# LeoQLi/DeepSIR

Hardware: AMD Instinct MI355X
Metric: registered pairs/sec (5k-pt 3DMatch-shaped synthetic pairs, 5 registration iterations, KNN pyramid included) (higher is better)
Workload: dtype f32 (GEMMs as fp16-pair MFMA, fp32 accumulate; index decisions exact fp32)

## Files before the change

### deepsir_amd/_lib.py

```python
from __future__ import annotations

import ctypes as C
import os

_HERE = os.path.dirname(os.path.abspath(__file__))
LIB_PATH = os.environ.get("DSIR_LIB", os.path.join(_HERE, "libdsir.so"))

c_float_p = C.POINTER(C.c_float)
c_i32_p = C.POINTER(C.c_int32)
c_i64_p = C.POINTER(C.c_int64)


class dsir_cfg(C.Structure):
    _fields_ = [
        ("feat_len", C.c_int32),
        ("num_knn", C.c_int32),
        ("num_layers", C.c_int32),
        ("sub_sampling_ratio", C.c_int32 * 4),
        ("d_out", C.c_int32 * 4),
        ("out_feat_dim", C.c_int32),
        ("num_classes", C.c_int32),
        ("max_points", C.c_int32),
        ("max_pairs", C.c_int32),
        ("pipeline", C.c_int32),
# ... 39 lines not shown
        ("xyz", C.c_void_p), ("feat", C.c_void_p), ("logits", C.c_void_p), ("score", C.c_void_p), ("label", C.c_void_p),
        ("index", C.c_void_p),
    ]


SYMBOLS = {
    "dsir_create": (C.c_int, [C.c_int, C.POINTER(dsir_cfg), C.POINTER(C.c_void_p)]),
    "dsir_create_ex": (C.c_int, [C.c_int, C.POINTER(dsir_cfg), C.c_int, C.POINTER(C.c_void_p)]),
    "dsir_destroy": (None, [C.c_void_p]),
    "dsir_last_error": (C.c_char_p, [C.c_void_p]),
    "dsir_stream": (C.c_void_p, [C.c_void_p]),
    "dsir_sync": (C.c_int, [C.c_void_p]),
    "dsir_set_stream": (C.c_int, [C.c_void_p, C.c_void_p, C.c_int]),
    "dsir_num_weights": (C.c_int, [C.c_void_p]),
    "dsir_weight_name": (C.c_char_p, [C.c_void_p, C.c_int, c_i64_p]),
    "dsir_load_weight": (C.c_int, [C.c_void_p, C.c_char_p, C.c_void_p, c_i64_p, C.c_int]),
    "dsir_finalize_weights": (C.c_int, [C.c_void_p]),
    "dsir_narrow_i64": (C.c_int, [C.c_void_p, C.c_void_p, C.c_void_p, C.c_int64]),
    "dsir_knn_pyramid": (C.c_int, [C.c_void_p, C.c_void_p, C.c_int, C.c_int, C.c_int, C.c_void_p, C.c_void_p,
                                   C.c_void_p, C.c_void_p]),
    "dsir_randla_forward": (C.c_int, [C.c_void_p, C.c_int, C.c_void_p, C.c_int, C.c_int, C.c_int, C.c_void_p,
                                      C.c_void_p, C.c_void_p, C.c_void_p, C.c_void_p, C.c_void_p]),
    "dsir_lfa_enc2_probe": (C.c_int, [C.c_void_p, C.c_int, C.c_int, C.c_int, C.c_int, C.c_int, C.c_void_p, C.c_void_p, C.c_void_p, C.c_void_p]),
    "dsir_ppf_pre": (C.c_int, [C.c_void_p, C.c_int, C.c_void_p, C.c_int, C.c_void_p, C.c_int64, C.c_int, C.c_int, C.c_void_p]),
    "dsir_estimate_normals": (C.c_int, [C.c_void_p, C.c_void_p, C.c_int, C.c_void_p, C.c_int64, C.c_int, C.c_int, c_float_p, C.c_void_p,
                                        C.c_void_p]),
    "dsir_estimate_normals_csr": (C.c_int, [C.c_void_p, C.c_void_p, C.c_int, C.c_void_p, C.c_void_p, C.c_int, C.c_int, c_float_p, C.c_void_p,
                                            C.c_void_p]),
    "dsir_fpfh": (C.c_int, [C.c_void_p, C.c_void_p, C.c_int, C.c_void_p, C.c_void_p, C.c_int64, C.c_void_p, C.c_void_p, C.c_int, C.c_int,
                            C.c_void_p, C.c_int, C.c_void_p]),
    "dsir_iss_keypoints": (C.c_int, [C.c_void_p, C.c_void_p, C.c_int, C.c_void_p, C.c_void_p, C.c_void_p, C.c_void_p, C.c_int, C.c_int,
                                     C.c_double, C.c_double, C.c_int, C.c_void_p, C.c_void_p, C.c_void_p, C.c_void_p]),
    "dsir_score": (C.c_int, [C.c_void_p, C.c_void_p, C.c_void_p, C.c_void_p, C.c_int64, C.c_void_p, C.c_int64,
                             C.c_int, C.c_int, C.c_void_p, C.c_void_p]),
    "dsir_aggregate": (C.c_int, [C.c_void_p, C.c_void_p, C.c_int64, C.c_void_p, C.c_void_p, C.c_int, C.c_int,
                                 C.c_void_p]),
    "dsir_nn_match": (C.c_int, [C.c_void_p, C.c_void_p, C.c_void_p, C.c_int, C.c_int, C.c_int, C.c_void_p]),
    "dsir_nn_match_screened": (C.c_int, [C.c_void_p, C.c_void_p, C.c_void_p, C.c_int, C.c_int, C.c_int, C.c_void_p, c_i64_p]),
    "dsir_kabsch": (C.c_int, [C.c_void_p, C.c_void_p, C.c_void_p, C.c_void_p, C.c_int, C.c_int, C.c_void_p,
                              C.c_void_p]),
    "dsir_register": (C.c_int, [C.c_void_p, C.POINTER(dsir_pair_batch), C.c_int, C.POINTER(dsir_pair_result)]),
    "dsir_forward_pair": (C.c_int, [C.c_void_p, C.POINTER(dsir_pair_batch), C.c_int, C.POINTER(dsir_cloud_out),
                                    C.POINTER(dsir_cloud_out)]),
    "dsir_icp_refine": (C.c_int, [C.c_void_p, C.c_void_p, C.c_void_p, C.c_int, C.c_int, C.c_int, C.c_int, C.c_float, C.c_int,
                                  C.c_float, C.c_float, C.c_void_p, C.c_void_p, C.c_void_p]),
    "dsir_icp_refine_ex": (C.c_int, [C.c_void_p, C.c_void_p, C.c_void_p, C.c_int, C.c_int, C.c_int, C.c_int, C.c_float, C.c_int,
# ... 181 lines not shown
```

### deepsir_amd/csrc/build.py

```python
from __future__ import annotations

import os
import subprocess
import sys
from concurrent.futures import ThreadPoolExecutor

HERE = os.path.dirname(os.path.abspath(__file__))
PKG = os.path.dirname(HERE)
ROOT = os.path.dirname(PKG)
SOURCES = ["engine.hip", "register.hip", "entries_stage.hip", "entries_pose.hip", "weights.hip", "schedule.hip", "search.hip", "pw_gemm.hip", "pw_stream.hip", "pw_tile.hip", "walk.hip", "att_pool.hip", "lse_uv.hip", "head_mlp.hip", "agg_chain.hip", "select.hip", "misc.hip", "knn.hip", "knn_grid.hip", "score.hip", "nn_match.hip", "nn_screen.hip", "nn_prune.hip", "kabsch.hip", "icp.hip", "icp_grid.hip", "finetune.hip", "pose_corr.hip", "ransac.hip", "consensus.hip", "fgr.hip", "align_loss.hip", "train_gemm.hip", "train_norm.hip", "train_gather.hip", "train_loss.hip", "train_elem.hip", "match_targets.hip", "metrics.hip", "preprocess.hip", "augment.hip", "crop.hip", "ppf.hip", "fpfh.hip", "iss.hip", "overlap.hip", "radius_nn.hip", "nn_topk.hip", "resample.hip", "seg_sort.hip", "info_matrix.hip", "pose_graph.hip"]
HEADERS = ["kernels.h", "device_utils.h", "svd3.h", "split_f16.h", "agg_chain_body.h", "head_mlp_body.h", "pw_tile_body.h", "att_pool_body.h", "misc_body.h", "ppf_plan.h", "search_plan.h", "screen_bound.h", "exact_search_body.h", "icp_plane.h", "icp_robust.h", "icp_grid.h", "icp_layout.h", "cell_index.h", "radius_nn.h", "scratch.h", "op_layouts.h", "train_ops.h", "train_layouts.h", "seg_sort.h", "augment_params.h", "pose_corr.h", "fgr.h", "engine_ctx.h", "pose_graph.h", os.path.join(ROOT, "include", "dsir.h"), os.path.join(ROOT, "include", "dsir_train.h")]
OUT = os.path.join(PKG, "libdsir.so")
FLAGS = ["--offload-arch=gfx950", "-O3", "-std=c++17", "-fPIC", "-ffp-contract=off", "-I" + os.path.join(ROOT, "include"),
         "-I" + HERE, "-Wall", "-Wno-unused-function", "-Wno-unused-value"]


def _newer(target, deps):
    if not os.path.exists(target):
        return False
    t = os.path.getmtime(target)
    return all(os.path.getmtime(d) <= t for d in deps)


def build(force: bool = False, verbose: bool = False) -> str:
    hipcc = os.environ.get("HIPCC", "/opt/rocm/bin/hipcc")
    objdir = os.path.join(HERE, "build")
    os.makedirs(objdir, exist_ok=True)
    hdrs = [h if os.path.isabs(h) else os.path.join(HERE, h) for h in HEADERS]
    jobs = []
    for s in SOURCES:
        src = os.path.join(HERE, s)
        obj = os.path.join(objdir, s.replace(".hip", ".o"))
        if force or not _newer(obj, [src] + hdrs):
# ... 28 lines not shown
```

### deepsir_amd/csrc/engine_ctx.h

```cpp
#pragma once
#include <hip/hip_runtime.h>

#include <string>
#include <unordered_map>
#include <vector>

#include "dsir.h"
#include "kernels.h"
#include "search_plan.h"

namespace dsir {

struct HostParam {
  std::string name;
  std::vector<int64_t> shape;
  std::vector<float> data;
  bool loaded = false;
  bool ignored = false;
  int64_t numel() const { int64_t n = 1; for (auto s : shape) n *= s; return n; }
};

struct Mlp2dW { const float *W = nullptr, *b = nullptr, *gamma = nullptr, *beta = nullptr; int cin = 0, cout = 0, groups = 0; };
struct AttW { const float* fc = nullptr; const float* fc_g = nullptr; int d = 0; Mlp2dW mlp; };
struct BlockW { Mlp2dW mlp1, lfa1, lfa2, mlp2, skip; AttW att1, att2; int d_in = 0, d = 0; const float* lse_w8 = nullptr;
// ... 178 lines not shown
struct EncCache {
  bool valid = false;
  float* s2_buf[DSIR_MAX_LEVELS][2] = {};
  float* enc_buf[DSIR_MAX_LEVELS] = {};
  float* uv_buf[DSIR_MAX_LEVELS] = {};
  float* dist_buf[DSIR_MAX_LEVELS] = {};
  float* enc2_buf[DSIR_MAX_LEVELS] = {};
  double* enc_stats[DSIR_MAX_LEVELS] = {};
  double* enc2_stats[DSIR_MAX_LEVELS] = {};
  Act enc[DSIR_MAX_LEVELS], enc2[DSIR_MAX_LEVELS];
  static size_t stats_words(const dsir_cfg& g, int P) { return (size_t)2 * g.num_layers * gn_layer_words(P); }
  int plan(dsir_ctx* c, const Pyramid& ps, double* prezeroed);
};

struct AggExtras { float* sq = nullptr; void* hi = nullptr; void* lo = nullptr; unsigned long long* packed_init = nullptr; };

void fill_pyramid_layout(const dsir_cfg& cfg, int clouds, int n, Pyramid& p);
int gn_max_contributions(const dsir_cfg& g, int n, int flags = 0);
int randla_forward(dsir_ctx* c, const RandlaW& w, const Seg& in0, const Seg* in1, const Pyramid& py, float* feat_out,
                   float* logits_out, EncCache* cache = nullptr);
int run_lfa_enc2_probe(dsir_ctx* c, const RandlaW& w, int level, int fused, const Pyramid& py, float* rows_out, double* stats_out);
int run_ppf_pre(dsir_ctx* c, const RandlaW& w, const float* rows, int stride, const int32_t* neigh, int64_t neigh_cs, int clouds, int n,
                float* out);
float* run_mlp_feat(dsir_ctx* c, const float* feat0, int clouds, int n, float* out = nullptr);
bool run_att_proj(dsir_ctx* c, const float* xyz, int64_t xyz_cs, const float* score, const float* F, int clouds, int n,
                  float* desc, const AggExtras* ex = nullptr);
int build_pyramid(dsir_ctx* c, const float* points, int stride, int clouds, int n, float* xyz, int32_t* neigh,
                  int32_t* sub, int32_t* interp);

void expect_state_dict(dsir_ctx* c);

struct DescSearch {
  dsir_ctx* c;
  SearchMode mode;
  int P, J, K;
  bool timed = false;
  bool counted = false;
  void* match_scratch = nullptr;
  void *ah = nullptr, *al = nullptr, *bh = nullptr, *bl = nullptr;
  float *sa = nullptr, *sb = nullptr;
  void* scratch = nullptr;
  void* prune_scratch = nullptr;
  unsigned long long* stats = nullptr;
  int32_t* bad = nullptr;
  AggExtras ex_ref, ex_src;
  const int32_t* prev_idx = nullptr;
  void alloc(bool with_match_scratch, bool with_stats = false, bool with_bad = false);
// ... 22 lines not shown
```

### deepsir_amd/csrc/entries_stage.hip

```cpp
#include <cmath>

#include "engine_ctx.h"

using namespace dsir;

extern "C" {

int dsir_narrow_i64(dsir_ctx* c, const int64_t* src, int32_t* dst, int64_t n) {
  Call call(c); if (call.refused()) return 1;
  launch_narrow_i64(src, dst, n, c->stream);
  return call.finish();
}

int dsir_knn_pyramid(dsir_ctx* c, const float* points, int stride, int clouds, int n, float* xyz, int32_t* neigh,
                     int32_t* sub, int32_t* interp) {
  Call call(c); if (call.refused()) return 1;
  if (clouds < 1 || stride < 3) return fail(c, "dsir_knn_pyramid: bad arguments");
  if (int r = build_pyramid(c, points, stride, clouds, n, xyz, neigh, sub, interp)) return r;
  return call.finish();
}

int dsir_randla_forward(dsir_ctx* c, int which, const float* features, int cin, int clouds, int n, const float* xyz,
                        const int32_t* neigh, const int32_t* sub, const int32_t* interp, float* feat, float* logits) {
  Call call(c, Call::kWeights); if (call.refused()) return 1;
// ... 5 lines not shown
  if (check_batch(c, "randla_forward", clouds, n)) return 1;
  Pyramid py;
  fill_pyramid_layout(c->cfg, clouds, n, py);
  if (py.nl[3] < kKnn) return fail(c, "cloud too small (n=%d)", n);
  py.xyz = xyz; py.neigh = neigh; py.sub = sub; py.interp = interp;
  const Seg in0 = plain_seg(features, (int64_t)n * cin, w.ppf ? 3 : cin, cin);
  const Seg in1 = plain_seg(features + 3, (int64_t)n * cin, 3, cin);
  if (int r = call.begin_walker()) return r;
  if (int r = randla_forward(c, w, in0, w.ppf ? &in1 : nullptr, py, feat, logits)) return r;
  return call.finish();
}

int dsir_lfa_enc2_probe(dsir_ctx* c, int which, int level, int fused, int clouds, int n, const float* xyz, const int32_t* neigh,
                        float* rows, double* stats) {
  Call call(c, Call::kWeights); if (call.refused()) return 1;
  if (which != 0 && c->cfg.pipeline != DSIR_PIPELINE_ALIGN) return fail(c, "dsir_lfa_enc2_probe: this context has no inlier_model (pipeline != align)");
  if (!xyz || !neigh || !rows || !stats || clouds < 1 || level < 0 || level >= c->cfg.num_layers) return fail(c, "dsir_lfa_enc2_probe: bad arguments");
  if (check_batch(c, "dsir_lfa_enc2_probe", clouds, n)) return 1;
  Pyramid py;
  fill_pyramid_layout(c->cfg, clouds, n, py);
  if (py.nl[c->cfg.num_layers - 1] < kKnn) return fail(c, "cloud too small (n=%d)", n);
  py.xyz = xyz; py.neigh = neigh;
  if (int r = run_lfa_enc2_probe(c, which == 0 ? c->net.feat : c->net.inl, level, fused, py, rows, stats)) return r;
  return call.finish();
}

int dsir_ppf_pre(dsir_ctx* c, int which, const float* rows, int stride, const int32_t* neigh, int64_t neigh_cs, int clouds, int n,
                 float* out) {
  Call call(c, Call::kWeights); if (call.refused()) return 1;
  if (!(c->flags & DSIR_FLAG_PPF)) return fail(c, "dsir_ppf_pre: the context was not created with DSIR_FLAG_PPF");
  if (which != 0 && c->cfg.pipeline != DSIR_PIPELINE_ALIGN) return fail(c, "dsir_ppf_pre: this context has no inlier_model (pipeline != align)");
  if (!rows || !neigh || !out || clouds < 1 || n < kKnn) return fail(c, "dsir_ppf_pre: bad arguments");
  if (stride < 6) return fail(c, "dsir_ppf_pre: rows of xyz + normal need at least 6 columns, got %d (reference RandLANet.py:325)", stride);
  if (check_batch(c, "dsir_ppf_pre", clouds, n)) return 1;
  if (int r = run_ppf_pre(c, which == 0 ? c->net.feat : c->net.inl, rows, stride, neigh, neigh_cs, clouds, n, out)) return r;
  return call.finish();
}

int dsir_estimate_normals(dsir_ctx* c, const float* points, int stride, const int32_t* neigh, int64_t neigh_cs, int clouds, int n,
                          const float* viewpoint, float* normals, int32_t* flags) {
  Call call(c); if (call.refused()) return 1;
  if (!points || !neigh || !normals || clouds < 1 || clouds > 65535 || n < 1 || stride < 3) return fail(c, "dsir_estimate_normals: bad arguments");
  const float v[3] = {viewpoint ? viewpoint[0] : 0.f, viewpoint ? viewpoint[1] : 0.f, viewpoint ? viewpoint[2] : 0.f};
  launch_estimate_normals(points, (int64_t)n * stride, stride, neigh, neigh_cs, n, clouds, v[0], v[1], v[2], normals, flags, c->stream);
  return call.finish();
}
// ... 120 lines not shown
```

### deepsir_amd/csrc/kernels.h

```cpp
#pragma once
#include <hip/hip_runtime.h>
#include <stdint.h>
#include <stdlib.h>

namespace dsir {

constexpr int kKnn = 16;

const char* tuning_env(const char* name);
inline bool tuning_flag(const char* name) { return tuning_env(name) != nullptr; }
inline long long tuning_int(const char* name, long long dflt) { const char* e = tuning_env(name); return e ? atoll(e) : dflt; }

#ifndef DSIR_GN_WORDS_DEFINED
#define DSIR_GN_WORDS_DEFINED
constexpr int kGnWords = 4;
#endif
struct GnRef {
  const double* stats;
  const float* gamma;
  const float* beta;
  int groups;
  double inv_count;
};

// ... 175 lines not shown
};
bool launch_head_mlp(const HeadArgs& a, bool split, hipStream_t st);

struct AggArgs {
  const float* xyz = nullptr; int64_t xyz_cs = 0;
  const float* score = nullptr;
  const float* F = nullptr;
  const float *W1 = nullptr, *b1 = nullptr;
  const float *W2 = nullptr, *b2 = nullptr;
  const float *W3 = nullptr, *b3 = nullptr;
  const float *W4 = nullptr, *b4 = nullptr;
  const float *W5 = nullptr, *b5 = nullptr;
  const float *W6 = nullptr, *b6 = nullptr;
  float* desc = nullptr;
  int n = 0, clouds = 0;
  float* sq = nullptr;
  void* hi = nullptr;
  void* lo = nullptr;
  unsigned long long* packed_init = nullptr;
  const void* Wh[5] = {nullptr, nullptr, nullptr, nullptr, nullptr};
  const void* Wl[5] = {nullptr, nullptr, nullptr, nullptr, nullptr};
};
bool launch_agg_chain(const AggArgs& a, bool split, hipStream_t st);
void split_weights_f16(const float* w, size_t n, uint16_t* hi, uint16_t* lo);

size_t topk_scratch_bytes(int clouds, int n);
int launch_topk(const float* score, int clouds, int n, int k, int32_t* idx_out, float* score_out, void* scratch, hipStream_t st);
size_t scatter_plan_scratch_bytes(int64_t total);
int launch_scatter_plan(const int32_t* idx, int m, int clouds, int n, int32_t* order, int32_t* offsets, void* scratch, hipStream_t st);
void launch_gather_rows(const float* in, int64_t in_cloud_stride, int ld, const int32_t* idx, int C, int m, int clouds, float* out,
                        hipStream_t st);
void launch_gather_i32(const int32_t* in, int64_t in_cloud_stride, const int32_t* idx, int m, int clouds, int32_t* out,
                       hipStream_t st);
void launch_l2norm64(const float* x, int64_t rows, float* y, hipStream_t st);

void launch_residual_combine(const float* a, GnRef ga, const float* b, GnRef gb, int C, int rows, int clouds,
                             float* y, hipStream_t st);
void launch_gather_max(const float* in, int64_t in_cloud_stride, const int32_t* idx, int64_t idx_cloud_stride, int C,
                       int rows_out, int clouds, float* out, hipStream_t st);

void launch_gather_max_combine(const float* a, GnRef ga, const float* b, GnRef gb, int rows_in, const int32_t* idx,
                               int64_t idx_cloud_stride, int C, int rows_out, int clouds, float* out, hipStream_t st);

struct GmcArgs {
  const float* a; GnRef ga; const float* b; GnRef gb; int rows_in; const int32_t* idx; int64_t idx_cs; int C, rows_out; float* out; int bpc;
};
// ... 238 lines not shown
```

### deepsir_amd/csrc/register.hip

```cpp
#include <cstring>

#include "engine_ctx.h"

using namespace dsir;

extern "C" {

struct PairStage {
  Pyramid ps, pr;
  float *feat_s, *feat_r, *logit_s, *logit_r, *score_s, *score_r;
  int32_t *label_s, *label_r;
  float *rxyz;
};
static int forward_pair_stage(dsir_ctx* c, const dsir_pair_batch* in, bool want_score, bool want_label, PairStage& S,
                              int32_t* invalid = nullptr, MemOps pre = MemOps()) {
  const dsir_cfg& g = c->cfg;
  const int P = in->pairs, J = in->n_src, K = in->n_ref, cin = g.feat_len;
  if (P < 1 || P > g.max_pairs) return fail(c, "pairs=%d outside [1,%d]", P, g.max_pairs);
  if (J > g.max_points || K > g.max_points) return fail(c, "cloud larger than max_points=%d", g.max_points);
  if (!in->points_src || !in->points_ref) return fail(c, "null point clouds");
  const bool have_py = in->src_xyz && in->src_neigh && in->src_sub && in->src_interp && in->ref_xyz && in->ref_neigh &&
                       in->ref_sub && in->ref_interp;
  const bool any_py = in->src_xyz || in->src_neigh || in->src_sub || in->src_interp || in->ref_xyz || in->ref_neigh ||
                      in->ref_sub || in->ref_interp;
// ... 120 lines not shown
  const float* pxyz = ps.xyz;

  float* desc_r = ws.get<float>((size_t)P * K * 64);
  float* desc_s = ws.get<float>((size_t)P * J * 64);
  float* F_s = ws.get<float>((size_t)P * J * 64);
  float* xyz_cur = ws.get<float>((size_t)P * J * 3);
  float* logits_it = ws.get<float>((size_t)P * J);
  int32_t* idx_it = ws.get<int32_t>((size_t)P * J);
  float* T_it = ws.get<float>((size_t)P * 12);
  static const long long screen_min = tuning_int("DSIR_SCREEN_MIN_WORK", kScreenMinWork);
  const SearchSwitches sw{c->screen_mode, c->prune_min_points, c->prune_min_rows, screen_min};
  DescSearch search{c, search_mode(sw, P, J, K, in->forced_idx != nullptr, nn_prune_supported(P, J, K)), P, J, K, true, true};
  search.alloc(true);
  const size_t kab_bytes = kabsch_part_bytes(P, J, c->kabsch_chunked_min);
  double* kab_part = kab_bytes ? ws.get<double>(kab_bytes / sizeof(double)) : nullptr;
  EncCache enc_cache;
  static const bool no_hoist = tuning_flag("DSIR_NO_HOIST");
  const bool hoist = !no_hoist && n_iter > 1;
  if (hoist)
    if (int r = enc_cache.plan(c, ps, cache_stats_at)) return r;
  if (ws.overflow) return overflow_fail(c, "workspace exhausted (raise max_points / max_pairs)");
  const size_t mark1 = ws.mark();
  {
    run_mlp_feat(c, feat_s, P, J, F_s);
    launch_copy_xyz(pxyz, (int64_t)ps.S * 3, 3, J, P, xyz_cur, (int64_t)J * 3, st);
    float* F_r = run_mlp_feat(c, feat_r, P, K);
    const bool ref_prepared = run_att_proj(c, rxyz, (int64_t)pr.S * 3, score_r, F_r, P, K, desc_r, search.ref_extras());
    if (out->desc_ref) HIP_OK(c, hipMemcpyAsync(out->desc_ref, desc_r, sizeof(float) * P * K * 64, hipMemcpyDeviceToDevice, st));
    if (int r = search.prepare_ref(desc_r, ref_prepared, rxyz, (int64_t)pr.S * 3)) return r;
    ws.release(mark1);
  }

  for (int it = 0; it < n_iter; ++it) {
    int32_t* idx_out = out->idx ? out->idx + (size_t)it * P * J : idx_it;
    float* logit_out = out->logits ? out->logits + (size_t)it * P * J : logits_it;
    DescSearch::Iter si;
    si.it = it;
    si.src_prepared = run_att_proj(c, xyz_cur, (int64_t)J * 3, score_s, F_s, P, J, desc_s, search.src_extras());
    ws.release(mark1);
    if (out->desc_src)
      HIP_OK(c, hipMemcpyAsync(out->desc_src + (size_t)it * P * J * 64, desc_s, sizeof(float) * P * J * 64, hipMemcpyDeviceToDevice, st));
    if (in->forced_idx) { si.forced = in->forced_idx + (size_t)it * P * J; si.invalid = out->invalid; }
    if (int r = search.run(desc_s, desc_r, idx_out, si)) return r;
    const Seg s0 = plain_seg(xyz_cur, (int64_t)J * 3, 3, 3);
    const Seg s1 = plain_seg(rxyz, (int64_t)pr.S * 3, 3, 3, idx_out, J);
    if (int r = randla_forward(c, c->net.inl, s0, &s1, ps, nullptr, logit_out, hoist ? &enc_cache : nullptr)) return r;
    ws.release(mark1);
    KabschArgs a{};
    a.src = xyz_cur; a.ref = rxyz; a.idx = idx_out; a.w = logit_out; a.src_stride = (int64_t)J * 3; a.ref_stride = (int64_t)pr.S * 3;
// ... 166 lines not shown
```

### deepsir_amd/csrc/schedule.hip

```cpp
#include <cstddef>
#include <cstring>
#include <vector>

#include "engine_ctx.h"

namespace dsir {

namespace {
void level_sizes(const dsir_cfg& cfg, int n, int* nl) {
  nl[0] = n;
  for (int l = 0; l < cfg.num_layers; ++l) nl[l + 1] = nl[l] / cfg.sub_sampling_ratio[l];
}
}

void fill_pyramid_layout(const dsir_cfg& cfg, int clouds, int n, Pyramid& p) {
  p.clouds = clouds; p.n = n;
  level_sizes(cfg, n, p.nl);
  p.off[0] = 0; p.soff[0] = 0;
  for (int l = 0; l < cfg.num_layers; ++l) { p.off[l + 1] = p.off[l] + p.nl[l]; p.soff[l + 1] = p.soff[l] + p.nl[l + 1]; }
  p.S = p.off[cfg.num_layers]; p.S1 = p.soff[cfg.num_layers];
}

int gn_max_contributions(const dsir_cfg& g, int n, int flags) {
  const bool ppf = (flags & DSIR_FLAG_PPF) != 0;
// ... 547 lines not shown
    h.in = Sched::seg_of(x);
    h.W1 = w.out_w; h.W2 = w.fc[0].W; h.b2 = w.fc[0].b; h.W3 = w.fc[1].W; h.b3 = w.fc[1].b; h.W4 = w.fc[2].W; h.b4 = w.fc[2].b;
    h.ncls = w.ncls; h.M = n0; h.clouds = py.clouds; h.feat_out = feat_out; h.logits_out = logits_out;
    if (c->ws.overflow) return overflow_fail(c, "workspace exhausted in randla_forward (raise max_points / max_pairs)");
    if (c->agg_split) {
      for (int k = 0; k < 4; ++k) { h.Wh[k] = w.head_wh[k]; h.Wl[k] = w.head_wl[k]; }
      fused = launch_head_mlp(h, true, st);
    }
    if (!fused) fused = launch_head_mlp(h, false, st);
  }
  LinW ow; ow.W = w.out_w; ow.b = nullptr; ow.cin = w.dec_out; ow.cout = g.out_feat_dim;
  Act feat;
  if (!fused) feat = s.linear(ow, Sched::seg_of(x), nullptr, n0, EPI_LINEAR, feat_out);
  if (logits_out && !fused) {
    Act h = s.linear(w.fc[0], Sched::seg_of(feat), nullptr, n0, EPI_ACT);
    h = s.linear(w.fc[1], Sched::seg_of(h), nullptr, n0, EPI_ACT);
    s.linear(w.fc[2], Sched::seg_of(h), nullptr, n0, EPI_LINEAR, logits_out);
  }
  if (c->ws.overflow) return overflow_fail(c, "workspace exhausted in randla_forward (raise max_points / max_pairs)");
  if (cache) cache->valid = true;
  return 0;
}

float* run_mlp_feat(dsir_ctx* c, const float* feat0, int clouds, int n, float* out) {
  Sched s{c, c->stream, clouds};
  const NetW& w = c->net;
  Act h = s.linear(w.mlp_feat[0], plain_seg(feat0, (int64_t)n * 64, 64, 64), nullptr, n, EPI_ACT);
  h = s.linear(w.mlp_feat[1], Sched::seg_of(h), nullptr, n, EPI_ACT);
  h = s.linear(w.mlp_feat[2], Sched::seg_of(h), nullptr, n, EPI_LINEAR, out);
  return h.p;
}
bool run_att_proj(dsir_ctx* c, const float* xyz, int64_t xyz_cs, const float* score, const float* F, int clouds, int n,
                  float* desc, const AggExtras* ex) {
  Sched s{c, c->stream, clouds};
  const NetW& w = c->net;
  static const bool no_agg = tuning_flag("DSIR_NO_AGG");
  const LinW* m = w.mlp_att;
  if (!no_agg && m[0].cin == 4 && m[0].cout == 32 && m[1].cout == 64 && m[2].cout == 128 && m[3].cout == 256 &&
      m[4].cout == 64 && w.mlp_proj.cin == 64 && w.mlp_proj.cout == 64) {
    AggArgs a;
    a.xyz = xyz; a.xyz_cs = xyz_cs; a.score = score; a.F = F;
    a.W1 = m[0].W; a.b1 = m[0].b; a.W2 = m[1].W; a.b2 = m[1].b; a.W3 = m[2].W; a.b3 = m[2].b;
    a.W4 = m[3].W; a.b4 = m[3].b; a.W5 = m[4].W; a.b5 = m[4].b; a.W6 = w.mlp_proj.W; a.b6 = w.mlp_proj.b;
    a.desc = desc; a.n = n; a.clouds = clouds;
    static const bool no_fuse = tuning_flag("DSIR_NO_AGG_EXTRAS");
    if (c->agg_split) {
      for (int k = 0; k < 5; ++k) { a.Wh[k] = c->agg_wh[k]; a.Wl[k] = c->agg_wl[k]; }
      if (ex && !no_fuse) { a.sq = ex->sq; a.hi = ex->hi; a.lo = ex->lo; a.packed_init = ex->packed_init; }
      if (launch_agg_chain(a, true, c->stream)) return ex && !no_fuse;
      a.sq = nullptr; a.hi = a.lo = nullptr; a.packed_init = nullptr;
    }
    if (launch_agg_chain(a, false, c->stream)) return false;
  }
// ... 84 lines not shown
```

### deepsir_amd/engine.py

```python
from __future__ import annotations

import ctypes as C
from typing import Dict, Optional, Sequence, Tuple

import numpy as np
import torch

from . import _lib
from .arch import PIPELINES, NetConfig, level_sizes


class EngineError(RuntimeError):
    pass


def check_pose_weight(w) -> float:
    w = float(w)
    if not (w >= 0.0) or w == float("inf"):
        raise EngineError(f"align_loss_backward: wt_pose_loss must be finite and >= 0, got {w}")
    return w


def _ptr(t: Optional[torch.Tensor]) -> Optional[int]:
    return None if t is None else t.data_ptr()
# ... 168 lines not shown
        xyz, neigh, sub, interp = (_chk(xyz, torch.float32, "xyz"), _chk(neigh, torch.int32, "neigh_idx"),
                                   _chk(sub, torch.int32, "sub_idx"), _chk(interp, torch.int32, "interp_idx"))
        self._pre()
        self._call(self.lib.dsir_randla_forward(self.h, w, _ptr(features), cin, c, n, _ptr(xyz), _ptr(neigh), _ptr(sub),
                                                _ptr(interp), _ptr(feat), _ptr(logits)))
        self.sync()
        return feat, logits

    def lfa_enc2_probe(self, which: str, level: int, fused: bool, xyz, neigh, n: int):
        xyz, neigh = _chk(xyz, torch.float32, "xyz"), _chk(neigh, torch.int32, "neigh_idx")
        c = xyz.shape[0]
        assert xyz.shape[1] == self.pyramid_shapes(n)[0]
        nl = n
        for r in self.cfg.sub_sampling_ratio[:level]:
            nl //= r
        ch = self.cfg.d_out[level] // 2
        rows = self._empty((c, 16 * nl, ch))
        stats = self._empty((c, 8 if ch >= 64 else 4, 4), torch.float64)
        self._pre()
        self._call(self.lib.dsir_lfa_enc2_probe(self.h, {"feat_extractor": 0, "inlier_model": 1}[which], level, int(fused), c, n, _ptr(xyz),
                                                _ptr(neigh), _ptr(rows), _ptr(stats)))
        self.sync()
        return rows, stats

    def ppf_pre(self, which: str, rows, neigh_multi):
        rows, neigh_multi = _chk(rows, torch.float32, "rows"), _chk(neigh_multi, torch.int32, "neigh_idx")
        c, n, stride = rows.shape
        out = self._empty((c, n, 12))
        self._pre()
        self._call(self.lib.dsir_ppf_pre(self.h, {"feat_extractor": 0, "inlier_model": 1}[which], _ptr(rows), stride, _ptr(neigh_multi),
                                         neigh_multi.shape[1] * 16, c, n, _ptr(out)))
        self.sync()
        return out

    def estimate_normals(self, points, neigh_multi=None, viewpoint=(0.0, 0.0, 0.0), csr=None):
        points = _chk(points, torch.float32, "points")
        if (neigh_multi is None) == (csr is None):
            raise EngineError("estimate_normals: exactly one of neigh_multi and csr expected")
        c, n, stride = points.shape
        normals = self._empty((c, n, 3))
        flags = self._empty((c, n), torch.int32)
        v = (C.c_float * 3)(*[float(x) for x in viewpoint])
        if csr is None:
            neigh_multi = _chk(neigh_multi, torch.int32, "neigh_idx")
            self._pre()
            self._call(self.lib.dsir_estimate_normals(self.h, _ptr(points), stride, _ptr(neigh_multi), neigh_multi.shape[1] * 16, c, n, v,
# ... 877 lines not shown
```

### include/dsir.h

```cpp
#ifndef DSIR_H
#define DSIR_H

#include <stdint.h>
#include <stddef.h>

#ifdef __cplusplus
extern "C" {
#endif

#define DSIR_MAX_LEVELS 4
#define DSIR_KNN 16

typedef struct dsir_ctx dsir_ctx;

typedef struct dsir_cfg {
  int32_t feat_len;
  int32_t num_knn;
  int32_t num_layers;
  int32_t sub_sampling_ratio[DSIR_MAX_LEVELS];
  int32_t d_out[DSIR_MAX_LEVELS];
  int32_t out_feat_dim;
  int32_t num_classes;
  int32_t max_points;
  int32_t max_pairs;
// ... 11 lines not shown
void dsir_destroy(dsir_ctx* ctx);
const char* dsir_last_error(const dsir_ctx* ctx);
void* dsir_stream(dsir_ctx* ctx);
int dsir_sync(dsir_ctx* ctx);
int dsir_set_stream(dsir_ctx* ctx, void* hip_stream, int restore_own);
int dsir_num_weights(const dsir_ctx* ctx);
const char* dsir_weight_name(const dsir_ctx* ctx, int i, int64_t* numel);

int dsir_load_weight(dsir_ctx* ctx, const char* key, const float* host_data, const int64_t* shape, int ndim);
int dsir_finalize_weights(dsir_ctx* ctx);


int dsir_narrow_i64(dsir_ctx* ctx, const int64_t* src, int32_t* dst, int64_t n);

int dsir_knn_pyramid(dsir_ctx* ctx, const float* points, int stride, int clouds, int n,
                     float* xyz_multi, int32_t* neigh_idx, int32_t* sub_idx, int32_t* interp_idx);

int dsir_randla_forward(dsir_ctx* ctx, int which, const float* features, int cin, int clouds, int n,
                        const float* xyz_multi, const int32_t* neigh_idx, const int32_t* sub_idx,
                        const int32_t* interp_idx, float* feat, float* logits);

int dsir_lfa_enc2_probe(dsir_ctx* ctx, int which, int level, int fused, int clouds, int n, const float* xyz_multi,
                        const int32_t* neigh_idx, float* rows, double* stats);

int dsir_ppf_pre(dsir_ctx* ctx, int which, const float* rows, int stride, const int32_t* neigh_idx, int64_t neigh_cloud_stride,
                 int clouds, int n, float* out);

int dsir_estimate_normals(dsir_ctx* ctx, const float* points, int stride, const int32_t* neigh_idx, int64_t neigh_cloud_stride,
                          int clouds, int n, const float* viewpoint, float* normals, int32_t* flags);
int dsir_estimate_normals_csr(dsir_ctx* ctx, const float* points, int stride, const int32_t* csr_offsets, const int32_t* csr_cols,
                              int clouds, int n, const float* viewpoint, float* normals, int32_t* flags);

int dsir_fpfh(dsir_ctx* ctx, const float* points, int stride, const float* normals, const int32_t* neigh_idx,
              int64_t neigh_cloud_stride, const int32_t* csr_offsets, const int32_t* csr_cols, int clouds, int n, float* desc,
              int out_ld, int32_t* flags);

int dsir_iss_keypoints(dsir_ctx* ctx, const float* points, int stride, const int32_t* sal_offsets, const int32_t* sal_cols,
                       const int32_t* nms_offsets, const int32_t* nms_cols, int clouds, int n, double gamma_21, double gamma_32,
                       int min_neighbors, float* saliency, int32_t* mask, int32_t* index, int32_t* counts);

int dsir_score(dsir_ctx* ctx, const float* feat, const float* logits, const float* xyz, int64_t xyz_cloud_stride,
               const int32_t* neigh_idx, int64_t neigh_cloud_stride, int clouds, int n, float* score, int32_t* label);

int dsir_aggregate(dsir_ctx* ctx, const float* xyz, int64_t xyz_cloud_stride, const float* feat0, const float* score,
                   int clouds, int n, float* desc);

// ... 225 lines not shown
```

Baseline: 5130.

## Fuse three-layer feature MLP into one persistent MFMA kernel, batching source and reference

Adds a persistent kernel that runs the 64→64→128→64 feature MLP in a single launch. Weights stay in LDS, intermediate activations stay in per-wave LDS scratch, and the input tile is prefetched. In registration, when the source and reference features sit next to each other, both clouds go through one launch with a split output pointer, where before there were six separate GEMM launches. The first two layers use fp32 MFMA, which may cost more than the previous fp16-split path, and the last layer keeps the split-f16 form.

```diff
diff --git a/deepsir_amd/_lib.py b/deepsir_amd/_lib.py
--- a/deepsir_amd/_lib.py
+++ b/deepsir_amd/_lib.py
@@ -85,6 +85,7 @@
     "dsir_randla_forward": (C.c_int, [C.c_void_p, C.c_int, C.c_void_p, C.c_int, C.c_int, C.c_int, C.c_void_p,
                                       C.c_void_p, C.c_void_p, C.c_void_p, C.c_void_p, C.c_void_p]),
     "dsir_lfa_enc2_probe": (C.c_int, [C.c_void_p, C.c_int, C.c_int, C.c_int, C.c_int, C.c_int, C.c_void_p, C.c_void_p, C.c_void_p, C.c_void_p]),
+    "dsir_mlp_feat_probe": (C.c_int, [C.c_void_p, C.c_void_p, C.c_int, C.c_int, C.c_int, C.c_int, C.c_void_p]),
     "dsir_ppf_pre": (C.c_int, [C.c_void_p, C.c_int, C.c_void_p, C.c_int, C.c_void_p, C.c_int64, C.c_int, C.c_int, C.c_void_p]),
     "dsir_estimate_normals": (C.c_int, [C.c_void_p, C.c_void_p, C.c_int, C.c_void_p, C.c_int64, C.c_int, C.c_int, c_float_p, C.c_void_p,
                                         C.c_void_p]),
diff --git a/deepsir_amd/csrc/build.py b/deepsir_amd/csrc/build.py
--- a/deepsir_amd/csrc/build.py
+++ b/deepsir_amd/csrc/build.py
@@ -8,7 +8,7 @@
 HERE = os.path.dirname(os.path.abspath(__file__))
 PKG = os.path.dirname(HERE)
 ROOT = os.path.dirname(PKG)
-SOURCES = ["engine.hip", "register.hip", "entries_stage.hip", "entries_pose.hip", "weights.hip", "schedule.hip", "search.hip", "pw_gemm.hip", "pw_stream.hip", "pw_tile.hip", "walk.hip", "att_pool.hip", "lse_uv.hip", "head_mlp.hip", "agg_chain.hip", "select.hip", "misc.hip", "knn.hip", "knn_grid.hip", "score.hip", "nn_match.hip", "nn_screen.hip", "nn_prune.hip", "kabsch.hip", "icp.hip", "icp_grid.hip", "finetune.hip", "pose_corr.hip", "ransac.hip", "consensus.hip", "fgr.hip", "align_loss.hip", "train_gemm.hip", "train_norm.hip", "train_gather.hip", "train_loss.hip", "train_elem.hip", "match_targets.hip", "metrics.hip", "preprocess.hip", "augment.hip", "crop.hip", "ppf.hip", "fpfh.hip", "iss.hip", "overlap.hip", "radius_nn.hip", "nn_topk.hip", "resample.hip", "seg_sort.hip", "info_matrix.hip", "pose_graph.hip"]
+SOURCES = ["engine.hip", "register.hip", "entries_stage.hip", "entries_pose.hip", "weights.hip", "schedule.hip", "search.hip", "pw_gemm.hip", "pw_stream.hip", "pw_tile.hip", "walk.hip", "att_pool.hip", "lse_uv.hip", "head_mlp.hip", "agg_chain.hip", "feat_chain.hip", "select.hip", "misc.hip", "knn.hip", "knn_grid.hip", "score.hip", "nn_match.hip", "nn_screen.hip", "nn_prune.hip", "kabsch.hip", "icp.hip", "icp_grid.hip", "finetune.hip", "pose_corr.hip", "ransac.hip", "consensus.hip", "fgr.hip", "align_loss.hip", "train_gemm.hip", "train_norm.hip", "train_gather.hip", "train_loss.hip", "train_elem.hip", "match_targets.hip", "metrics.hip", "preprocess.hip", "augment.hip", "crop.hip", "ppf.hip", "fpfh.hip", "iss.hip", "overlap.hip", "radius_nn.hip", "nn_topk.hip", "resample.hip", "seg_sort.hip", "info_matrix.hip", "pose_graph.hip"]
 HEADERS = ["kernels.h", "device_utils.h", "svd3.h", "split_f16.h", "agg_chain_body.h", "head_mlp_body.h", "pw_tile_body.h", "att_pool_body.h", "misc_body.h", "ppf_plan.h", "search_plan.h", "screen_bound.h", "exact_search_body.h", "icp_plane.h", "icp_robust.h", "icp_grid.h", "icp_layout.h", "cell_index.h", "radius_nn.h", "scratch.h", "op_layouts.h", "train_ops.h", "train_layouts.h", "seg_sort.h", "augment_params.h", "pose_corr.h", "fgr.h", "engine_ctx.h", "pose_graph.h", os.path.join(ROOT, "include", "dsir.h"), os.path.join(ROOT, "include", "dsir_train.h")]
 OUT = os.path.join(PKG, "libdsir.so")
 FLAGS = ["--offload-arch=gfx950", "-O3", "-std=c++17", "-fPIC", "-ffp-contract=off", "-I" + os.path.join(ROOT, "include"),
diff --git a/deepsir_amd/csrc/engine_ctx.h b/deepsir_amd/csrc/engine_ctx.h
--- a/deepsir_amd/csrc/engine_ctx.h
+++ b/deepsir_amd/csrc/engine_ctx.h
@@ -224,7 +224,10 @@
 int run_lfa_enc2_probe(dsir_ctx* c, const RandlaW& w, int level, int fused, const Pyramid& py, float* rows_out, double* stats_out);
 int run_ppf_pre(dsir_ctx* c, const RandlaW& w, const float* rows, int stride, const int32_t* neigh, int64_t neigh_cs, int clouds, int n,
                 float* out);
-float* run_mlp_feat(dsir_ctx* c, const float* feat0, int clouds, int n, float* out = nullptr);
+enum class FeatForm { Auto, Three, Fused };
+float* run_mlp_feat(dsir_ctx* c, const float* feat0, int clouds, int n, float* out = nullptr, FeatForm form = FeatForm::Auto, int max_blocks = 0);
+float* run_mlp_feat_pair(dsir_ctx* c, const float* feat0, int P, int n, float* out_a, FeatForm form = FeatForm::Auto, int max_blocks = 0);
+int run_mlp_feat_probe(dsir_ctx* c, const float* feat0, int clouds, int n, int fused, int max_blocks, float* out);
 bool run_att_proj(dsir_ctx* c, const float* xyz, int64_t xyz_cs, const float* score, const float* F, int clouds, int n,
                   float* desc, const AggExtras* ex = nullptr);
 int build_pyramid(dsir_ctx* c, const float* points, int stride, int clouds, int n, float* xyz, int32_t* neigh,
diff --git a/deepsir_amd/csrc/entries_stage.hip b/deepsir_amd/csrc/entries_stage.hip
--- a/deepsir_amd/csrc/entries_stage.hip
+++ b/deepsir_amd/csrc/entries_stage.hip
@@ -51,6 +51,15 @@
   if (py.nl[c->cfg.num_layers - 1] < kKnn) return fail(c, "cloud too small (n=%d)", n);
   py.xyz = xyz; py.neigh = neigh;
   if (int r = run_lfa_enc2_probe(c, which == 0 ? c->net.feat : c->net.inl, level, fused, py, rows, stats)) return r;
+  return call.finish();
+}
+
+int dsir_mlp_feat_probe(dsir_ctx* c, const float* feat0, int clouds, int n, int fused, int max_workgroups, float* out) {
+  Call call(c, Call::kWeights); if (call.refused()) return 1;
+  if (c->cfg.pipeline == DSIR_PIPELINE_LABEL) return fail(c, "dsir_mlp_feat_probe: a label-pipeline context has no aggregation layers");
+  if (!feat0 || !out || clouds < 1 || n < 1 || fused < 0 || fused > 2 || (fused == 2 && (clouds & 1)) || max_workgroups < 0) return fail(c, "dsir_mlp_feat_probe: bad arguments");
+  if (check_batch(c, "dsir_mlp_feat_probe", clouds, n)) return 1;
+  if (int r = run_mlp_feat_probe(c, feat0, clouds, n, fused, max_workgroups, out)) return r;
   return call.finish();
 }
 
diff --git a/deepsir_amd/csrc/feat_chain.hip b/deepsir_amd/csrc/feat_chain.hip
--- /dev/null
+++ b/deepsir_amd/csrc/feat_chain.hip
@@ -0,0 +1,201 @@
+#include <hip/hip_fp16.h>
+
+#include "kernels.h"
+#include "device_utils.h"
+#include "split_f16.h"
+
+namespace dsir {
+
+namespace {
+
+constexpr int kWaves = 8;
+constexpr int kDefaultCUs = 256;
+constexpr int W2_LD = 20;
+constexpr int T1_LD = 20;
+constexpr int T2_LD = 36;
+constexpr int W3_LD = 128 + 4;
+constexpr int T_WORDS = 4 * 16 * T2_LD;
+
+template <bool SPLIT>
+__global__ __launch_bounds__(64 * kWaves) void feat_chain_kernel(const FeatChainArgs p) {
+  __shared__ __attribute__((aligned(16))) float s_w2[4 * 128 * W2_LD];
+  __shared__ __attribute__((aligned(16))) float s_w3[SPLIT ? 2 * 16 * 64 * 4 : 64 * W3_LD];
+  __shared__ __attribute__((aligned(16))) float s_T[kWaves][T_WORDS];
+
+  const int tid = threadIdx.x, lane = tid & 63, w = __builtin_amdgcn_readfirstlane(tid >> 6);
+  const int fr = lane & 15, fq = lane >> 4;
+
+  float w1[4][16], b1[4], b2[8], b3[4];
+#pragma unroll
+  for (int t = 0; t < 4; ++t) {
+#pragma unroll
+    for (int i = 0; i < 4; ++i) {
+      const float4 v = *reinterpret_cast<const float4*>(p.W1 + (16 * t + fr) * 64 + 16 * fq + 4 * i);
+      w1[t][4 * i] = v.x; w1[t][4 * i + 1] = v.y; w1[t][4 * i + 2] = v.z; w1[t][4 * i + 3] = v.w;
+    }
+    b1[t] = p.b1 ? p.b1[16 * t + fr] : 0.f;
+    b3[t] = p.b3 ? p.b3[16 * t + fr] : 0.f;
+  }
+#pragma unroll
+  for (int t = 0; t < 8; ++t) b2[t] = p.b2 ? p.b2[16 * t + fr] : 0.f;
+
+  for (int i = tid; i < 128 * 16; i += 64 * kWaves) {
+    const int col = i >> 4, q4 = i & 15;
+    *reinterpret_cast<float4*>(&s_w2[((q4 >> 2) * 128 + col) * W2_LD + 4 * (q4 & 3)]) = *reinterpret_cast<const float4*>(p.W2 + col * 64 + 4 * q4);
+  }
+  if constexpr (SPLIT) {
+    const uint4* gh = reinterpret_cast<const uint4*>(p.W3h);
+    const uint4* gl = reinterpret_cast<const uint4*>(p.W3l);
+    uint4* d = reinterpret_cast<uint4*>(s_w3);
+    for (int i = tid; i < 64 * 16; i += 64 * kWaves) {
+      const int col = i >> 4, u = i & 15;
+      d[u * 64 + col] = gh[i];
+      d[(16 + u) * 64 + col] = gl[i];
+    }
+  } else {
+    for (int i = tid; i < 64 * 32; i += 64 * kWaves) {
+      const int col = i >> 5, c4 = i & 31;
+      *reinterpret_cast<float4*>(&s_w3[col * W3_LD + 4 * c4]) = *reinterpret_cast<const float4*>(p.W3 + col * 128 + 4 * c4);
+    }
+  }
+  __syncthreads();
+
+  float* T = s_T[w];
+  const int ntiles = (p.n + 15) >> 4;
+  const int total = p.clouds * ntiles, stride = gridDim.x * kWaves;
+
+  float4 x[4], xn[4];
+  auto load_x = [&](int g, float4 (&v)[4]) {
+    const int cloud = g / ntiles, tile = g - cloud * ntiles;
+    const int row = min(tile * 16 + fr, p.n - 1);
+    const float* src = p.X + ((int64_t)cloud * p.n + row) * 64 + 16 * fq;
+#pragma unroll
+    for (int i = 0; i < 4; ++i) v[i] = *reinterpret_cast<const float4*>(src + 4 * i);
+  };
+  int g = blockIdx.x * kWaves + w;
+  if (g < total) load_x(g, x);
+  for (; g < total; g += stride) {
+    if (g + stride < total) load_x(g + stride, xn);
+    const int cloud = g / ntiles, tile = g - cloud * ntiles;
+
+    f32x4 c1[4];
+#pragma unroll
+    for (int t = 0; t < 4; ++t) c1[t] = f32x4{0.f, 0.f, 0.f, 0.f};
+#pragma unroll
+    for (int i = 0; i < 4; ++i) {
+      const float a[4] = {x[i].x, x[i].y, x[i].z, x[i].w};
+#pragma unroll
+      for (int j = 0; j < 4; ++j)
+#pragma unroll
+        for (int t = 0; t < 4; ++t) c1[t] = __builtin_amdgcn_mfma_f32_16x16x4f32(a[j], w1[t][4 * i + j], c1[t], 0, 0, 0);
+    }
+    __builtin_amdgcn_wave_barrier();
+#pragma unroll
+    for (int t = 0; t < 4; ++t)
+#pragma unroll
+      for (int r = 0; r < 4; ++r) {
+        float v = c1[t][r] + b1[t];
+        if (v < 0.f) v *= 0.2f;
+        T[(t * 16 + 4 * fq + r) * T1_LD + fr] = v;
+      }
+    __builtin_amdgcn_wave_barrier();
+    float4 a1[4];
+#pragma unroll
+    for (int i = 0; i < 4; ++i) a1[i] = *reinterpret_cast<const float4*>(&T[(fq * 16 + fr) * T1_LD + 4 * i]);
+
+    f32x4 c2[8];
+#pragma unroll
+    for (int t = 0; t < 8; ++t) c2[t] = f32x4{0.f, 0.f, 0.f, 0.f};
+#pragma unroll
+    for (int i = 0; i < 4; ++i) {
+      float4 b[8];
+#pragma unroll
+      for (int t = 0; t < 8; ++t) b[t] = *reinterpret_cast<const float4*>(&s_w2[(fq * 128 + 16 * t + fr) * W2_LD + 4 * i]);
+      const float a[4] = {a1[i].x, a1[i].y, a1[i].z, a1[i].w};
+#pragma unroll
+      for (int j = 0; j < 4; ++j)
+#pragma unroll
+        for (int t = 0; t < 8; ++t) {
+          const float bj = j == 0 ? b[t].x : (j == 1 ? b[t].y : (j == 2 ? b[t].z : b[t].w));
+          c2[t] = __builtin_amdgcn_mfma_f32_16x16x4f32(a[j], bj, c2[t], 0, 0, 0);
+        }
+    }
+    __builtin_amdgcn_wave_barrier();
+#pragma unroll
+    for (int t = 0; t < 8; ++t)
+#pragma unroll
+      for (int r = 0; r < 4; ++r) {
+        float v = c2[t][r] + b2[t];
+        if (v < 0.f) v *= 0.2f;
+        T[((2 * (t & 1) + (fr >> 3)) * 16 + 4 * fq + r) * T2_LD + 8 * (t >> 1) + (fr & 7)] = v;
+      }
+    __builtin_amdgcn_wave_barrier();
+
+    f32x4 c3[4];
+#pragma unroll
+    for (int t = 0; t < 4; ++t) c3[t] = f32x4{0.f, 0.f, 0.f, 0.f};
+    if constexpr (SPLIT) {
+      h8 ah[4], al[4];
+#pragma unroll
+      for (int s = 0; s < 4; ++s) {
+        const float4* q = reinterpret_cast<const float4*>(&T[(fq * 16 + fr) * T2_LD + 8 * s]);
+        split8(q[0], q[1], ah[s], al[s]);
+      }
+      const h8* wh = reinterpret_cast<const h8*>(s_w3);
+#pragma unroll
+      for (int t = 0; t < 4; ++t)
+#pragma unroll
+        for (int s = 0; s < 4; ++s)
+          mma3(c3[t], ah[s], al[s], wh[(4 * s + fq) * 64 + 16 * t + fr], wh[(16 + 4 * s + fq) * 64 + 16 * t + fr]);
+    } else {
+#pragma unroll
+      for (int S = 0; S < 32; ++S) {
+        const float a = T[(((S & 7) >> 1) * 16 + fr) * T2_LD + 8 * (S >> 3) + 4 * (S & 1) + fq];
+#pragma unroll
+        for (int t = 0; t < 4; ++t)
+          c3[t] = __builtin_amdgcn_mfma_f32_16x16x4f32(a, s_w3[(16 * t + fr) * W3_LD + 4 * S + fq], c3[t], 0, 0, 0);
+      }
+    }
+    float* Y = cloud < p.split_cloud ? p.out0 + (int64_t)cloud * p.n * 64 : p.out1 + (int64_t)(cloud - p.split_cloud) * p.n * 64;
+    const int rbase = tile * 16 + 4 * fq;
+#pragma unroll
+    for (int t = 0; t < 4; ++t)
+#pragma unroll
+      for (int r = 0; r < 4; ++r)
+        if (rbase + r < p.n) Y[(int64_t)(rbase + r) * 64 + 16 * t + fr] = c3[t][r] + b3[t];
+#pragma unroll
+    for (int i = 0; i < 4; ++i) x[i] = xn[i];
+  }
+}
+
+}
+
+long long feat_chain_blocks(int clouds, int n) { return ((long long)clouds * ((n + 15) / 16) + kWaves - 1) / kWaves; }
+
+bool launch_feat_chain(const FeatChainArgs& a, hipStream_t st) {
+  if (a.n <= 0 || a.clouds <= 0) return true;
+  static const bool other = tuning_flag("DSIR_NO_STREAM") || tuning_flag("DSIR_NO_TILE") || tuning_int("DSIR_TILE_MIN_COUT", 32) > 64;
+  if (other) return false;
+  if (!a.X || !a.W1 || !a.W2 || !a.W3 || !a.out0 || (a.split_cloud < a.clouds && !a.out1) || a.split_cloud < 0) return false;
+  if ((reinterpret_cast<uintptr_t>(a.X) | reinterpret_cast<uintptr_t>(a.W1) | reinterpret_cast<uintptr_t>(a.W2) |
+       reinterpret_cast<uintptr_t>(a.W3)) % 16)
+    return false;
+  static const bool tile_f32 = tuning_flag("DSIR_TILE_F32");
+  const bool split = a.W3h && a.W3l && !tile_f32;
+  if (split && (reinterpret_cast<uintptr_t>(a.W3h) | reinterpret_cast<uintptr_t>(a.W3l)) % 16) return false;
+  const int64_t total = (int64_t)a.clouds * ((a.n + 15) / 16);
+  if (total > 0x7fffffffll - 64 * 1024) return false;
+  static const int cus = [] {
+    int dev = 0, n = 0;
+    const bool ok = hipGetDevice(&dev) == hipSuccess && hipDeviceGetAttribute(&n, hipDeviceAttributeMultiprocessorCount, dev) == hipSuccess;
+    return ok && n > 0 ? n : kDefaultCUs;
+  }();
+  const int64_t want = feat_chain_blocks(a.clouds, a.n);
+  const int64_t most = a.max_blocks > 0 && a.max_blocks < cus ? a.max_blocks : cus;
+  const int blocks = (int)(want < most ? want : most);
+  if (split) hipLaunchKernelGGL(feat_chain_kernel<true>, dim3(blocks), dim3(64 * kWaves), 0, st, a);
+  else hipLaunchKernelGGL(feat_chain_kernel<false>, dim3(blocks), dim3(64 * kWaves), 0, st, a);
+  return true;
+}
+
+}
diff --git a/deepsir_amd/csrc/kernels.h b/deepsir_amd/csrc/kernels.h
--- a/deepsir_amd/csrc/kernels.h
+++ b/deepsir_amd/csrc/kernels.h
@@ -221,6 +221,21 @@
   const void* Wl[5] = {nullptr, nullptr, nullptr, nullptr, nullptr};
 };
 bool launch_agg_chain(const AggArgs& a, bool split, hipStream_t st);
+
+struct FeatChainArgs {
+  const float* X = nullptr;
+  const float *W1 = nullptr, *b1 = nullptr;
+  const float *W2 = nullptr, *b2 = nullptr;
+  const float *W3 = nullptr, *b3 = nullptr;
+  const void *W3h = nullptr, *W3l = nullptr;
+  float* out0 = nullptr;
+  float* out1 = nullptr;
+  int split_cloud = 0;
+  int n = 0, clouds = 0;
+  int max_blocks = 0;
+};
+bool launch_feat_chain(const FeatChainArgs& a, hipStream_t st);
+long long feat_chain_blocks(int clouds, int n);
 void split_weights_f16(const float* w, size_t n, uint16_t* hi, uint16_t* lo);
 
 size_t topk_scratch_bytes(int clouds, int n);
diff --git a/deepsir_amd/csrc/register.hip b/deepsir_amd/csrc/register.hip
--- a/deepsir_amd/csrc/register.hip
+++ b/deepsir_amd/csrc/register.hip
@@ -166,9 +166,14 @@
   if (ws.overflow) return overflow_fail(c, "workspace exhausted (raise max_points / max_pairs)");
   const size_t mark1 = ws.mark();
   {
-    run_mlp_feat(c, feat_s, P, J, F_s);
+    float* F_r;
+    if (J == K && feat_r == feat_s + (size_t)P * J * 64) {
+      F_r = run_mlp_feat_pair(c, feat_s, P, J, F_s);
+    } else {
+      run_mlp_feat(c, feat_s, P, J, F_s);
+      F_r = run_mlp_feat(c, feat_r, P, K);
+    }
     launch_copy_xyz(pxyz, (int64_t)ps.S * 3, 3, J, P, xyz_cur, (int64_t)J * 3, st);
-    float* F_r = run_mlp_feat(c, feat_r, P, K);
     const bool ref_prepared = run_att_proj(c, rxyz, (int64_t)pr.S * 3, score_r, F_r, P, K, desc_r, search.ref_extras());
     if (out->desc_ref) HIP_OK(c, hipMemcpyAsync(out->desc_ref, desc_r, sizeof(float) * P * K * 64, hipMemcpyDeviceToDevice, st));
     if (int r = search.prepare_ref(desc_r, ref_prepared, rxyz, (int64_t)pr.S * 3)) return r;
diff --git a/deepsir_amd/csrc/schedule.hip b/deepsir_amd/csrc/schedule.hip
--- a/deepsir_amd/csrc/schedule.hip
+++ b/deepsir_amd/csrc/schedule.hip
@@ -593,13 +593,68 @@
   return 0;
 }
 
-float* run_mlp_feat(dsir_ctx* c, const float* feat0, int clouds, int n, float* out) {
+namespace {
+bool feat_chain_wanted(int clouds, int n) {
+  static const bool off = tuning_flag("DSIR_NO_FEAT_CHAIN");
+  static const long long min_blocks = tuning_int("DSIR_FEAT_CHAIN_MIN_BLOCKS", 64);
+  return !off && feat_chain_blocks(clouds, n) >= min_blocks;
+}
+bool mlp_feat_chain(dsir_ctx* c, const float* feat0, int clouds, int n, float* out0, float* out1, int split_cloud, int max_blocks) {
+  const LinW* m = c->net.mlp_feat;
+  if (m[0].cin != 64 || m[0].cout != 64 || m[1].cin != 64 || m[1].cout != 128 || m[2].cin != 128 || m[2].cout != 64) return false;
+  FeatChainArgs a;
+  a.X = feat0;
+  a.W1 = m[0].W; a.b1 = m[0].b; a.W2 = m[1].W; a.b2 = m[1].b; a.W3 = m[2].W; a.b3 = m[2].b;
+  GemmArgs last;
+  last.W = m[2].W;
+  Sched{c, c->stream, clouds}.split_of(last);
+  a.W3h = last.Wh; a.W3l = last.Wl;
+  a.out0 = out0; a.out1 = out1; a.split_cloud = split_cloud; a.n = n; a.clouds = clouds; a.max_blocks = max_blocks;
+  return launch_feat_chain(a, c->stream);
+}
+bool takes_fused(FeatForm form, int clouds, int n) { return form == FeatForm::Fused || (form == FeatForm::Auto && feat_chain_wanted(clouds, n)); }
+}
+
+float* run_mlp_feat(dsir_ctx* c, const float* feat0, int clouds, int n, float* out, FeatForm form, int max_blocks) {
   Sched s{c, c->stream, clouds};
   const NetW& w = c->net;
+  if (takes_fused(form, clouds, n)) {
+    float* y = out ? out : c->ws.get<float>((size_t)clouds * n * 64);
+    if (c->ws.overflow) return y;
+    if (mlp_feat_chain(c, feat0, clouds, n, y, nullptr, clouds, max_blocks)) return y;
+    if (form == FeatForm::Fused) return nullptr;
+    out = y;
+  }
   Act h = s.linear(w.mlp_feat[0], plain_seg(feat0, (int64_t)n * 64, 64, 64), nullptr, n, EPI_ACT);
   h = s.linear(w.mlp_feat[1], Sched::seg_of(h), nullptr, n, EPI_ACT);
   h = s.linear(w.mlp_feat[2], Sched::seg_of(h), nullptr, n, EPI_LINEAR, out);
   return h.p;
+}
+float* run_mlp_feat_pair(dsir_ctx* c, const float* feat0, int P, int n, float* out_a, FeatForm form, int max_blocks) {
+  float* out_b = c->ws.get<float>((size_t)P * n * 64);
+  if (c->ws.overflow) return out_b;
+  if (takes_fused(form, 2 * P, n) && mlp_feat_chain(c, feat0, 2 * P, n, out_a, out_b, P, max_blocks)) return out_b;
+  if (form == FeatForm::Fused) return nullptr;
+  run_mlp_feat(c, feat0, P, n, out_a, FeatForm::Three);
+  run_mlp_feat(c, feat0 + (size_t)P * n * 64, P, n, out_b, FeatForm::Three);
+  return out_b;
+}
+int run_mlp_feat_probe(dsir_ctx* c, const float* feat0, int clouds, int n, int fused, int max_blocks, float* out) {
+  if (fused == 2) {
+    const int P = clouds / 2;
+    const float* half = run_mlp_feat_pair(c, feat0, P, n, out, FeatForm::Fused, max_blocks);
+    if (c->ws.overflow) return overflow_fail(c, "workspace exhausted in mlp_feat_probe");
+    if (!half) return fail(c, "mlp_feat_probe: the fused launch does not take this configuration");
+    HIP_OK(c, hipMemcpyAsync(out + (size_t)P * n * 64, half, sizeof(float) * P * n * 64, hipMemcpyDeviceToDevice, c->stream));
+    return 0;
+  }
+  const float* y = run_mlp_feat(c, feat0, clouds, n, out, fused ? FeatForm::Fused : FeatForm::Three, max_blocks);
+  if (c->ws.overflow) {
+    if (c->call.sched_error) return fail(c, "mlp_feat_probe: %s", c->call.sched_error);
+    return overflow_fail(c, "workspace exhausted in mlp_feat_probe");
+  }
+  if (!y) return fail(c, "mlp_feat_probe: the fused launch does not take this configuration");
+  return 0;
 }
 bool run_att_proj(dsir_ctx* c, const float* xyz, int64_t xyz_cs, const float* score, const float* F, int clouds, int n,
                   float* desc, const AggExtras* ex) {
diff --git a/deepsir_amd/engine.py b/deepsir_amd/engine.py
--- a/deepsir_amd/engine.py
+++ b/deepsir_amd/engine.py
@@ -214,6 +214,16 @@
                                                 _ptr(neigh), _ptr(rows), _ptr(stats)))
         self.sync()
         return rows, stats
+
+    def mlp_feat_probe(self, feat0, fused: int, max_workgroups: int = 0):
+        feat0 = _chk(feat0, torch.float32, "feat0")
+        c, n, ch = feat0.shape
+        assert ch == 64
+        out = self._empty((c, n, 64))
+        self._pre()
+        self._call(self.lib.dsir_mlp_feat_probe(self.h, _ptr(feat0), c, n, int(fused), int(max_workgroups), _ptr(out)))
+        self.sync()
+        return out
 
     def ppf_pre(self, which: str, rows, neigh_multi):
         rows, neigh_multi = _chk(rows, torch.float32, "rows"), _chk(neigh_multi, torch.int32, "neigh_idx")
diff --git a/include/dsir.h b/include/dsir.h
--- a/include/dsir.h
+++ b/include/dsir.h
@@ -57,6 +57,8 @@
 
 int dsir_lfa_enc2_probe(dsir_ctx* ctx, int which, int level, int fused, int clouds, int n, const float* xyz_multi,
                         const int32_t* neigh_idx, float* rows, double* stats);
+
+int dsir_mlp_feat_probe(dsir_ctx* ctx, const float* feat0, int clouds, int n, int fused, int max_workgroups, float* out);
 
 int dsir_ppf_pre(dsir_ctx* ctx, int which, const float* rows, int stride, const int32_t* neigh_idx, int64_t neigh_cloud_stride,
                  int clouds, int n, float* out);
```

Result: faster. 5211 (median of 6 runs) (+1.6%).
